# It4innovations/hyperqueue

Hardware: AMD Instinct MI355X
Metric: tasks_assigned_per_sec (higher is better)
Workload: dtype u64

## Files before the change

### hyperqueue_amd/csrc/debug_capi.cpp

```cpp
#include "../../include/hqtick_debug.h"

#include <algorithm>
#include <cstring>

#include "audit_core.h"
#include "cancel_core.h"
#include "clock_core.h"
#include "fail_core.h"
#include "finish_core.h"
#include "lose_core.h"
#include "start_core.h"
#include "reject_core.h"
#include "hb_order.h"
#include "milp.h"
#include "price_emul.h"

static thread_local int g_last_canonical = 0;
static thread_local long g_last_hull[2] = {0, 0};
extern "C" int hqtick_debug_milp_was_canonical(void) { return g_last_canonical; }
extern "C" void hqtick_debug_milp_last_hull(long *solves, long *nonpacking) {
    if (solves) *solves = g_last_hull[0];
    if (nonpacking) *nonpacking = g_last_hull[1];
}

// ... 37 lines not shown
    m.rhs.assign(rhs, rhs + nrows);
    m.roff.assign(row_off, row_off + nrows + 1);
    int nnz = nrows ? row_off[nrows] : 0;
    m.rcol.assign(row_col, row_col + nnz);
    m.rcoef.assign(row_coef, row_coef + nnz);
    if (col_group) m.col_group.assign(col_group, col_group + ncols);
    if (row_implied) m.row_implied.assign(row_implied, row_implied + nrows);
    hqprice::EmulatedSweeper emu;
    if (min_cols) emu.min_cols = min_cols;
    hqmilp::Result r = hqmilp::solve(m, time_limit_s, true, hqmilp::REFERENCE_MIP_REL_GAP, use_sweeps ? &emu : nullptr);
    g_last_canonical = r.canonical ? 1 : 0;
    g_last_hull[0] = r.hull_solves; g_last_hull[1] = r.hull_solves_nonpacking;
    if (stats_out) { stats_out[0] = r.price_sweeps; stats_out[1] = r.price_rounds; stats_out[2] = r.price_total_us; stats_out[3] = r.canonical ? 1.0 : 0.0; }
    if (!r.feasible) return 0;
    for (int j = 0; j < ncols; j++) x_out[j] = r.x[j];
    *obj_out = r.objective;
    *is_optimal = r.optimal ? 1 : 0;
    return 1;
}

static thread_local hqmilp::Probe g_block_run_probe;
extern "C" void hqtick_debug_set_block_runs(int on) {
    hqmilp::g_probe = on < 0 ? nullptr : &g_block_run_probe; hqmilp::set_block_runs(on);
    if (on >= 0) { g_block_run_probe.model = g_block_run_probe.tables = g_block_run_probe.runs = g_block_run_probe.covered = 0; }
}
extern "C" void hqtick_debug_corrupt_block_runs(int on) { g_block_run_probe.corrupt_runs = on != 0; }
extern "C" void hqtick_debug_last_coupled_digest(uint64_t out[4]) {
    out[0] = g_block_run_probe.model; out[1] = g_block_run_probe.tables; out[2] = g_block_run_probe.runs; out[3] = g_block_run_probe.covered;
}
extern "C" void hqtick_debug_set_early_sweep(int on) { hqprice::set_early_sweep(on); }
extern "C" uint32_t hqtick_debug_early_sweeps(void) { return hqprice::early_sweeps(); }
extern "C" void hqtick_debug_capture_first_cut(int on) { hqprice::capture_first_cut(on != 0); }
extern "C" uint32_t hqtick_debug_first_cut(unsigned char *out, uint32_t cap) {
    const std::vector<unsigned char> &b = hqprice::first_cut_bytes();
    if (out && cap) memcpy(out, b.data(), std::min<size_t>(cap, b.size()));
    return (uint32_t)b.size();
}

static thread_local hqmilp::CheckHook g_row_check_hook;
static hqmilp::CheckHook &row_check_hook() { hqmilp::g_check_hook = &g_row_check_hook; return g_row_check_hook; }
extern "C" void hqtick_debug_set_defer_row_check(int on) { row_check_hook().allow = on; }
extern "C" uint32_t hqtick_debug_deferred_row_checks(int clear) { hqmilp::CheckHook &h = row_check_hook(); const uint32_t n = h.deferred; if (clear) h.deferred = 0; return n; }
extern "C" uint32_t hqtick_debug_fail_row_checks(uint32_t n) { hqmilp::CheckHook &h = row_check_hook(); const uint32_t left = h.fail_next; h.fail_next = n; return left; }

extern "C" int hqtick_debug_clock_rows(uint32_t n, const int64_t *deadline_ns, int64_t now_ns, uint32_t nv, const uint64_t *min_time_ns, int sorted_form, int64_t *remaining_out) {
    if ((n && (!deadline_ns || !remaining_out)) || (nv && !min_time_ns)) return HQTICK_E_INVALID;
    if (!sorted_form) {
        for (uint32_t w = 0; w < n; w++) {
            if (deadline_ns[w] == hqclock::NO_LIMIT) { remaining_out[w] = hqclock::NO_LIMIT; continue; }
            const int64_t r = hqclock::sat_sub(deadline_ns[w], now_ns);
            uint64_t best = 0;
            for (uint32_t v0 = 0; r >= 0 && v0 < nv; v0 += hqclock::CHUNK) best = hqclock::fold_thresholds(best, r, min_time_ns + v0, std::min(hqclock::CHUNK, nv - v0));
// ... 97 lines not shown
```

### hyperqueue_amd/csrc/host_model.cpp

```cpp
#include "host_model.h"

#include <algorithm>
#include <chrono>
#include <cmath>
#include <cstring>
#include <string>
#include <unordered_map>

#include "hb_order.h"

namespace hqhost {

namespace {

struct OrderEntry { uint64_t hash = 0; bool used = false; std::vector<uint32_t> ids, order; };
thread_local OrderEntry order_cache[32];
thread_local unsigned order_next = 0;
const std::vector<uint32_t> &cached_worker_order(const std::vector<uint32_t> &ids) {
    typedef OrderEntry Entry;
    Entry (&cache)[32] = order_cache;
    unsigned &next = order_next;
    uint64_t h = 0x9E3779B97F4A7C15ull ^ ids.size();
    for (uint32_t v : ids) { h ^= v; h *= 0xFF51AFD7ED558CCDull; h ^= h >> 29; }
    for (Entry &e : cache) if (e.used && e.hash == h && e.ids.size() == ids.size() && (ids.empty() || memcmp(e.ids.data(), ids.data(), ids.size() * 4) == 0)) return e.order;
// ... 1204 lines not shown
                    list_row(hqmilp::ROW_MAX, (double)cut.size, no_gap_id, *no_gap, -1, 0.0);
                }
            }
        }
    }

    if (!seq_start.empty()) {
        m.start.assign(m.ncols(), 0.0);
        for (const SeqStart &ss : seq_start) {
            const int pc = place_get(ss.w, batches[ss.batch].rq, ss.variant);
            if (pc < 0) { m.start.clear(); break; }
            m.start[pc] = ss.count;
        }
    }
    m.row_implied.resize(m.nrows(), 0);
    m.row_lhs.resize((size_t)m.nrows(), -1); m.row_lhs_len.resize((size_t)m.nrows(), 0); m.row_block.resize((size_t)m.nrows(), -1);
    m.col_ub = col_ub; m.col_ub.resize((size_t)m.ncols(), UINT32_MAX);
    if (hqmilp::g_probe) {
        using hqmilp::fnv1a_vec;
        uint64_t h = hqmilp::FNV_BASIS;
        h = fnv1a_vec(h, m.obj); h = fnv1a_vec(h, m.kind); h = fnv1a_vec(h, m.rtype); h = fnv1a_vec(h, m.rhs); h = fnv1a_vec(h, m.roff); h = fnv1a_vec(h, m.rcol); h = fnv1a_vec(h, m.rcoef);
        h = fnv1a_vec(h, m.start); h = fnv1a_vec(h, m.col_group); h = fnv1a_vec(h, m.row_implied); h = fnv1a_vec(h, m.row_lhs); h = fnv1a_vec(h, m.row_lhs_len);
        h = fnv1a_vec(h, m.list_off); h = fnv1a_vec(h, m.list_col); h = fnv1a_vec(h, m.row_block); h = fnv1a_vec(h, m.col_ub);
        hqmilp::g_probe->model = h; hqmilp::g_probe->runs = m.block_runs.size(); hqmilp::g_probe->tables = 0; hqmilp::g_probe->covered = 0;
    }
    const double t_model1 = clock_us();
    if (trace_model) {
        size_t run_blocks = 0; for (const auto &br : m.block_runs) run_blocks += (size_t)br.n_blocks;
        fprintf(stderr, "[model] cuts done at %.3f ms: %d columns, %d rows, %zu terms, %zu worker signatures, %zu (batch, cut, blocker) passes over the workers; %zu equal-block runs over %zu blocks, %zu (cut, blocker) passes decided once\n", (t_model1 - t_model0) / 1e3, m.ncols(), m.nrows(), m.rcol.size(), sig_rep.size(), n_triples, m.block_runs.size(), run_blocks, n_decided_once);
    }
    hqmilp::SolveOpts opts; opts.no_fast_path = pb.no_fast_path; opts.defer_row_check = pb.defer_row_check;
    hqmilp::Result sol = hqmilp::solve(m, pb.time_limit_s, !pb.certificate_only, hqmilp::REFERENCE_MIP_REL_GAP, pb.pricer, &opts);
    if (trace_model) fprintf(stderr, "[model] solve done %.3f ms after the model\n", (clock_us() - t_model1) / 1e3);
    out.pre_us = t_model0 - t_enter; out.model_us = t_model1 - t_model0; out.milp_us = clock_us() - t_model1; out.price_sweeps = sol.price_sweeps; out.price_rounds = sol.price_rounds; out.price_us = sol.price_total_us;
    out.milp_nodes = sol.nodes; out.milp_cols = m.ncols(); out.milp_rows = m.nrows(); out.milp_components = sol.n_components;
    if (!sol.feasible) return out;
    out.is_optimal = sol.optimal;
    out.is_canonical = sol.canonical && sol.optimal;

    std::vector<uint64_t> key_hash; std::vector<std::pair<uint32_t, uint8_t>> key_list; std::vector<std::vector<std::pair<uint32_t, uint32_t>>> key_counts;
    std::vector<uint64_t> mn_hash; std::vector<uint32_t> mn_list; std::vector<std::vector<std::vector<uint32_t>>> mn_sets;
    std::vector<uint32_t> dec_ids, dec_widx, dec_cnt;
    for (const TaskBatch &batch : batches) {
        const RequestView &rv = pb.rqs[batch.rq];
        if (pb.rq_multi_node(batch.rq)) {
            size_t n_nodes = pb.variants[rv.first_variant].n_nodes;
            std::vector<std::vector<uint32_t>> sets;
// ... 42 lines not shown
```

### hyperqueue_amd/csrc/milp.cpp

```cpp
#include "milp.h"
#include "lp_tab.h"
#include "price.h"

#include <algorithm>
#include <chrono>
#include <cstdio>
#include <cstdlib>
#include <cmath>
#include <climits>
#include <cstring>
#include <functional>
#include <numeric>
#include <string>
#include <unordered_map>

namespace hqmilp {
namespace {

using namespace lp;

struct DSUlite {
    std::vector<int> p;
    explicit DSUlite(int n) : p(n) { std::iota(p.begin(), p.end(), 0); }
    int find(int a) { while (p[a] != a) { p[a] = p[p[a]]; a = p[a]; } return a; }
// ... 1336 lines not shown
    rc.pending = false;
    if (g_check_hook && g_check_hook->fail_next > 0) { g_check_hook->fail_next--; return false; }
    return check_point(m, rc.x, rc.cost_scale, rc.bound, rc.rel_gap, &rc.objective);
}

namespace {
bool solve_fast(const Model &mdl_in, double time_limit_s, double rel_gap, hqprice::Sweeper *sweeper, const double ts0, const SolveOpts *opts, Result &res_out) {
    static const bool tracing_solve = getenv("HQMILP_TRACE") != nullptr;
    auto tmark = [&](const char *what) { if (tracing_solve && mdl_in.ncols() > 1000) fprintf(stderr, "[milp] solve(): %s at %.3f ms\n", what, (wall() - ts0) * 1e3); };
    static const bool fast_env = !(getenv("HQMILP_FAST") && atoi(getenv("HQMILP_FAST")) == 0);
    const bool fast_on = !(opts && opts->no_fast_path) && (g_fast_path < 0 ? fast_env : g_fast_path != 0);
    const int FAST_MIN_COLS = 2048;
    const bool hints_there = (int)mdl_in.col_group.size() == mdl_in.ncols() && (int)mdl_in.row_lhs.size() == mdl_in.nrows() && (int)mdl_in.row_lhs_len.size() == mdl_in.nrows();
    const bool takes_it = fast_on && sweeper && rel_gap > 0.0 && mdl_in.ncols() >= FAST_MIN_COLS && mdl_in.ncols() >= (int)sweeper->min_cols && hints_there && (int)mdl_in.start.size() != mdl_in.ncols();
    if (takes_it || (g_probe && hints_there)) {
        const int n = mdl_in.ncols(), m = mdl_in.nrows();
        hqprice::ModelView mv;
        mv.n = n; mv.m = m; mv.obj = mdl_in.obj.data(); mv.kind = mdl_in.kind.data(); mv.rtype = mdl_in.rtype.data(); mv.rhs = mdl_in.rhs.data();
        mv.roff = mdl_in.roff.data(); mv.rcol = mdl_in.rcol.data(); mv.rcoef = mdl_in.rcoef.data(); mv.col_group = mdl_in.col_group.data();
        mv.row_implied = (int)mdl_in.row_implied.size() == m ? mdl_in.row_implied.data() : nullptr; mv.row_lhs = mdl_in.row_lhs.data(); mv.row_lhs_len = mdl_in.row_lhs_len.data(); mv.list_off = mdl_in.list_off.data(); mv.list_col = mdl_in.list_col.data(); mv.n_lists = (int)mdl_in.list_off.size() - 1;
        if ((int)mdl_in.row_block.size() == m && (int)mdl_in.col_ub.size() == n) { mv.row_block = mdl_in.row_block.data(); mv.col_ub = mdl_in.col_ub.data(); }
        static_assert(sizeof(Model::BlockRun) == 7 * sizeof(int32_t), "ModelView::block_runs reads seven int32 per run");
        if (!mdl_in.block_runs.empty()) { mv.block_runs = &mdl_in.block_runs[0].col0; mv.n_block_runs = (int)mdl_in.block_runs.size(); }
        mv.run_stats = g_probe ? &g_probe->covered : nullptr; mv.tables_digest = g_probe ? &g_probe->tables : nullptr;
        if (!takes_it) { hqprice::flatten_for_probe(mv, tracing_solve); return false; }
        double cost_scale = 1.0;
        const double tf0 = wall();
        hqprice::Answer pa = hqprice::solve_model(mv, rel_gap, time_limit_s, ts0 + (time_limit_s > 0 ? time_limit_s : 1e18), tracing_solve, *sweeper, &cost_scale);
        if (tracing_solve) fprintf(stderr, "[milp] fast path: ran %d (%s) sweeps %u rounds %u bound %.9f point %.9f, %.3f ms of which %.3f ms inside the sweeps\n", (int)pa.ran, pa.why, pa.sweeps, pa.rounds, pa.ran ? pa.bound : -1.0, pa.x.empty() ? -1.0 : pa.x_value, (wall() - tf0) * 1e3, sweeper->stat_sweep_us / 1e3);
        if (pa.ran && (int)pa.x.size() == n && pa.bound * (1.0 + 1e-9) + 1e-12 <= pa.x_value + rel_gap * std::fabs(pa.x_value)) {
            if (opts && opts->defer_row_check) {
                Result res;
                res.x.resize((size_t)n);
                for (int j = 0; j < n; j++) res.x[(size_t)j] = std::floor(pa.x[(size_t)j] + 0.5);
                res.feasible = true; res.optimal = true; res.canonical = false;
                res.n_components = 1; res.nodes = pa.sweeps; res.price_sweeps = (int)pa.sweeps; res.price_rounds = (int)pa.rounds; res.price_total_us = (wall() - tf0) * 1e6;
                res.row_check.pending = true; res.row_check.x = std::move(pa.x); res.row_check.cost_scale = cost_scale; res.row_check.bound = pa.bound; res.row_check.rel_gap = rel_gap;
                if (g_check_hook) g_check_hook->deferred++;
                tmark("fast path certified by the sweeps, row check pending");
                res_out = std::move(res);
                return true;
            }
            double z_pt = 0.0;
            const bool ok = check_point(mdl_in, pa.x, cost_scale, pa.bound, rel_gap, &z_pt);
            if (ok) {
                Result res;
                res.x = std::move(pa.x);
// ... 301 lines not shown
```

### hyperqueue_amd/csrc/milp.h

```cpp
#pragma once
#include <cstddef>
#include <cstdint>
#include <algorithm>
#include <vector>

namespace hqprice { struct Sweeper; }

namespace hqmilp {

enum { COL_NAT = 0, COL_BOOL = 1 };
enum { ROW_MIN = 0, ROW_MAX = 1, ROW_EQ = 2 };

struct Model {
    std::vector<double> obj;
    std::vector<uint8_t> kind;
    std::vector<uint8_t> rtype;
    std::vector<double> rhs;
    std::vector<int> roff{0};
    std::vector<int> rcol;
    std::vector<double> rcoef;
    std::vector<double> start;
    std::vector<int32_t> col_group;
    std::vector<uint8_t> row_implied;
    std::vector<int32_t> row_lhs, row_lhs_len;
// ... 60 lines not shown
    int n_components = 0;
    int price_sweeps = 0, price_rounds = 0;
    double price_bound_us = 0, price_total_us = 0;
    long hull_solves = 0, hull_solves_nonpacking = 0;
    RowCheck row_check;
};

struct SolveOpts {
    bool no_fast_path = false;
    bool defer_row_check = false;
};

const double REFERENCE_MIP_REL_GAP = 1e-4;

Result solve(const Model &m, double time_limit_s, bool canonical = true, double rel_gap = REFERENCE_MIP_REL_GAP, hqprice::Sweeper *sweeper = nullptr, const SolveOpts *opts = nullptr);

bool check_point(const Model &m, const std::vector<double> &x, double cost_scale, double bound, double rel_gap, double *objective);
bool run_row_check(const Model &m, RowCheck &rc);

void columns_by_cost_desc(const double *c, int n, std::vector<int> &out);
void set_fast_path(int on);
void set_block_runs(int on);
bool block_runs_on();
struct Probe { uint64_t model = 0, tables = 0, runs = 0, covered = 0; bool corrupt_runs = false; };
extern thread_local Probe *g_probe;
struct CheckHook { int allow = -1; uint32_t deferred = 0, fail_next = 0; };
extern thread_local CheckHook *g_check_hook;
inline uint64_t fnv1a(uint64_t h, const void *p, size_t bytes) { const unsigned char *b = (const unsigned char *)p; for (size_t i = 0; i < bytes; i++) h = (h ^ b[i]) * 1099511628211ull; return h; }
template <class T> inline uint64_t fnv1a_vec(uint64_t h, const std::vector<T> &v) { const uint64_t n = v.size(); h = fnv1a(h, &n, 8); return v.empty() ? h : fnv1a(h, v.data(), v.size() * sizeof(T)); }
const uint64_t FNV_BASIS = 1469598103934665603ull;

}
```

### hyperqueue_amd/csrc/price.cpp

```cpp
#include "price_prob.h"

#include <algorithm>
#include <chrono>
#include <cmath>
#include <cstdio>
#include <cstdlib>
#include <cstring>
#include <functional>
#include <map>
#include <numeric>

#include "lp_tab.h"
#include "milp.h"

namespace hqprice {
namespace {

using hqmilp::lp::BASIC;
using hqmilp::lp::INF;
using hqmilp::lp::LP_OPT;
using hqmilp::lp::Rows;
using hqmilp::lp::Tab;

static_assert(UNBOUNDED == INF, "price_prob.h restates lp_tab.h's INF");
// ... 649 lines not shown
        out.lambda.assign(cuts.size(), 0.0); out.bfrac.assign(G, 0.0);
        double lsum = 0.0;
        for (int r = 0; r < M.m; r++) {
            const int a = mt.where[r];
            if (a < 0 || mt.st[M.n + a] == BASIC) continue;
            const double v = std::fabs(mt.d[M.n + a]) / row_scale[r];
            if (row_cut[r] >= 0) { out.lambda[row_cut[r]] = v; lsum += v; } else out.bfrac[freeg[r]] = std::min(1.0, v);
        }
        for (int g = 0; g < G; g++) if (nd.flag[g] >= 0) out.bfrac[g] = (double)nd.flag[g];
        if (lsum > 0.0) for (double &l : out.lambda) l /= lsum; else out.lambda.clear();
        out.pi.assign(mt.x.begin(), mt.x.begin() + K);
    }
};

}

namespace {
thread_local bool g_capture_cut = false; thread_local std::vector<unsigned char> g_first_cut;
Answer run_solver(Solver &S, const double tp0) {
    Answer ans;
    const Request &rq = S.rq; Sweeper &sw = S.sw;
    auto tmark = [&](const char *what) { if (rq.trace) fprintf(stderr, "[price] %s at %.3f ms (sweeps so far %.3f ms)\n", what, (now_us() - tp0) / 1e3, sw.stat_sweep_us / 1e3); };
    tmark("model flattened");
    if (rq.trace) fprintf(stderr, "[price]   %d equal-block runs took %d of %u blocks from their first one\n", S.P.n_runs, S.P.run_blocks, S.P.T.n_blocks);
    Prob &P = S.P;
    if (rq.trace) fprintf(stderr, "[price] %u blocks, %u block columns, %d wide rows with %d distinct left-hand sides (%zu / %zu terms), %d flags, %zu conditional bounds\n", P.T.n_blocks, P.T.n_cols, P.K, P.KG, P.row_terms, P.T.w_row.size(), P.G, P.caps.size());
    const int K = P.K, G = P.G;
    struct Ender { Sweeper *s; ~Ender() { if (s) s->end(); } } ender{S.early_begun ? &sw : nullptr};
    std::vector<double> pi0(K, 0.0);
    if (S.early == Solver::EARLY_REFUSED) { ans.why = "sweeper refused the model"; return ans; }
    if (S.early == Solver::EARLY_FAILED) { S.failed = true; ans.why = "sweep failed"; return ans; }
    if (S.early == Solver::EARLY_LAUNCHED) {
        if (!sw.begin_wide()) { ans.why = "sweeper refused the model"; return ans; }
        tmark("wide tables handed to the sweeper");
    } else {
        S.prepare_sweeper();
        if (!sw.begin(P.T, (uint32_t)S.max_sweeps)) { ans.why = "sweeper refused the model"; return ans; }
        ender.s = &sw;
        tmark("tables handed to the sweeper");
        if (!S.evaluate_launch(pi0)) { ans.why = "sweep failed"; return ans; }
    }
    S.pmax.assign(K, 0.0);
    {
        double cmax = 0.0; for (double c : P.T.col_cost) cmax = std::max(cmax, c);
        std::vector<double> gp(P.KG, 0.0);
        for (int g = 0; g < P.KG; g++) {
            double p = 0.0; bool neg = false; int32_t amin = INT32_MAX;
// ... 344 lines not shown
```

### hyperqueue_amd/csrc/price.h

```cpp
#pragma once
#include <cstdint>
#include <functional>
#include <vector>

namespace hqprice {

struct HostTables {
    uint32_t n_blocks = 0, n_cols = 0, K = 0;
    std::vector<uint32_t> blk_off; std::vector<uint8_t> blk_m; std::vector<double> blk_cap;
    std::vector<double> col_cost, col_a; std::vector<int32_t> col_cap; std::vector<uint32_t> col_woff; std::vector<uint16_t> w_row; std::vector<int32_t> w_coef;
};

struct SweepTotals {
    double cx = 0, rc = 0, bnd = 0;
    uint32_t n_budget = 0, max_steps = 0;
    std::vector<long long> act;
    std::vector<double> part_cx;
    std::vector<long long> part_act;
};
constexpr int PARTS = 16;

struct RangeValues { const double *cx = nullptr, *rc = nullptr, *bnd = nullptr; const uint32_t *steps = nullptr; const long long *part_act = nullptr; };

void totals_from_blocks(uint32_t n_blocks, uint32_t K, const double *cx, const double *rc, const double *bnd, const uint32_t *steps, const long long *part_act, SweepTotals &out);
// ... 39 lines not shown
    bool ran = false;
    double bound = 1e300;
    std::vector<double> x;
    double x_value = 0.0;
    uint32_t sweeps = 0, rounds = 0;
    const char *why = "";
    std::vector<int> block_of; std::vector<double> block_value, rcost;
};

Answer solve(const Request &rq, Sweeper &sw);

struct ModelView {
    int n = 0, m = 0;
    const double *obj = nullptr; const uint8_t *kind = nullptr;
    const uint8_t *rtype = nullptr; const double *rhs = nullptr;
    const int *roff = nullptr, *rcol = nullptr; const double *rcoef = nullptr;
    const int32_t *col_group = nullptr; const uint8_t *row_implied = nullptr;
    const int32_t *row_lhs = nullptr, *row_lhs_len = nullptr;
    const int *list_off = nullptr, *list_col = nullptr; int n_lists = 0;
    const int32_t *row_block = nullptr; const uint32_t *col_ub = nullptr;
    const int32_t *block_runs = nullptr; int n_block_runs = 0;
    uint64_t *run_stats = nullptr;
    uint64_t *tables_digest = nullptr;
};
void set_check_hints(bool on);
int hint_mismatches();
void set_early_sweep(int on);
uint32_t early_sweeps();
void capture_first_cut(bool on);
const std::vector<unsigned char> &first_cut_bytes();
void flatten_for_probe(const ModelView &mv, bool trace);
Answer solve_model(const ModelView &mv, double rel_gap, double time_limit_s, double deadline_s, bool trace, Sweeper &sw, double *cost_scale);

struct Exchange {
    uint32_t rank = 0, world = 1;
    virtual ~Exchange() {}
    virtual bool allgather(const void *send, void *recv, size_t bytes) = 0;
    uint64_t n_calls = 0, n_bytes = 0; double us = 0;
};

struct ShardedSweeper : Sweeper {
    Sweeper &inner; Exchange &ex;
    const HostTables *T = nullptr;
    std::vector<uint32_t> rank_b0, rank_b1, rank_p0, rank_p1;
    uint32_t max_blocks = 0, max_parts = 0, max_cols = 0;
    std::vector<unsigned char> send, recv;
    std::vector<double> cx, rc, bnd; std::vector<uint32_t> steps; std::vector<long long> part_act;
// ... 16 lines not shown
```

### hyperqueue_amd/csrc/price_flatten.cpp

```cpp
#include "price_prob.h"

#include <cstdio>
#include <cstring>

#include "milp.h"

namespace hqprice {
namespace {

constexpr double INF = UNBOUNDED;
thread_local bool g_check_hints = false; thread_local int g_hint_mismatches = 0;

#define HQ_PER_ROW inline __attribute__((always_inline))

typedef std::vector<std::pair<int, int32_t>> Lhs;

void finish_groups(Prob &P, const std::vector<Lhs> &lhs) {
    HostTables &T = P.T;
    const int KG = P.KG;
    T.K = (uint32_t)KG;
    size_t tot = 0; for (auto &l : lhs) tot += l.size();
    P.g_off.assign((size_t)KG + 1, 0); P.g_col.resize(tot); P.g_coef.resize(tot);
    std::vector<uint32_t> gcnt(T.n_cols + 1, 0);
    {
        auto *gc = P.g_col.data(); auto *gk = P.g_coef.data(); uint32_t *cnt = gcnt.data() + 1; size_t pos = 0;
        for (int g = 0; g < KG; g++) {
            const std::pair<int, int32_t> *l = lhs[(size_t)g].data();
            for (size_t i = 0, e = lhs[(size_t)g].size(); i < e; i++) { gc[pos] = l[i].first; gk[pos] = l[i].second; cnt[l[i].first]++; pos++; }
            P.g_off[(size_t)g + 1] = (int)pos;
        }
    }
    T.col_woff.assign(T.n_cols + 1, 0);
    for (uint32_t f = 0; f < T.n_cols; f++) T.col_woff[f + 1] = T.col_woff[f] + gcnt[f + 1];
    T.w_row.resize(T.col_woff[T.n_cols]); T.w_coef.resize(T.col_woff[T.n_cols]);
    {
        std::vector<uint32_t> &cur = gcnt;
        for (uint32_t f = 0; f < T.n_cols; f++) cur[f] = T.col_woff[f];
        uint32_t *cp = cur.data(); uint16_t *wr = T.w_row.data(); auto *wc = T.w_coef.data();
        const auto *gc = P.g_col.data(); const auto *gk = P.g_coef.data();
        for (int g = 0; g < KG; g++) for (int e = P.g_off[g], e1 = P.g_off[g + 1]; e < e1; e++) { const uint32_t p = cp[gc[e]]++; wr[p] = (uint16_t)g; wc[p] = gk[e]; }
    }
    P.gr_off.assign((size_t)KG + 1, 0);
    for (int k = 0; k < P.K; k++) P.gr_off[P.grp_of[k] + 1]++;
    for (int g = 0; g < KG; g++) P.gr_off[g + 1] += P.gr_off[g];
    P.gr_row.resize(P.K);
    { std::vector<int> c2(P.gr_off.begin(), P.gr_off.end() - 1); for (int k = 0; k < P.K; k++) P.gr_row[c2[P.grp_of[k]]++] = k; }
}

struct Scan { int b0 = -2; bool multi = false, has_g = false, nonneg = true; int n_bcols = 0; double amax = 0.0; };
struct Row { int a = 0, e = 0; bool is_le = false, is_ge = false, implied = false; double lo = 0.0, hi = 0.0; int list = -1, list_len = 0; Scan sc; };
struct WideRow { double h; uint8_t ge; int lhs_key; int own = -1; std::vector<std::pair<int, double>> g; };

template <class Rnd> HQ_PER_ROW const char *grid_terms(const double *coef, int nt, double scale, Rnd rnd, long long *vi, long long &g) {
    g = 0;
    for (int k = 0; k < nt; k++) {
        const double v = coef[k] * scale * GRID, rv = rnd(v);
        if (rv < 1.0 || std::fabs(v - rv) > 1e-6 * std::max(1.0, rv) || rv >= 4.0e15) return "block row off the ResourceAmount grid";
        vi[k] = (long long)rv;
        g = gcd_ll(g, vi[k]);
    }
    return nullptr;
}

struct Core {
    Prob &P; HostTables &T;
    const int n; const int32_t *const col_group; const int *const rcol; const double *const rcoef;
    const double *ub = nullptr, *c = nullptr;
    int max_group = -1, nb = 0;
    std::vector<int> block_of_group, bsize, blk, gidx;
    std::vector<WideRow> wide;
    std::vector<Lhs> own_lists;

    Core(Prob &p, int n_, const int32_t *cg, const int *rc, const double *rv) : P(p), T(p.T), n(n_), col_group(cg), rcol(rc), rcoef(rv) {}

    const char *number_blocks() {
        for (int j = 0; j < n; j++) max_group = std::max(max_group, col_group[j]);
        block_of_group.assign((size_t)max_group + 1, -1); blk.assign(n, -1);
        for (int j = 0; j < n; j++) {
            const int g = col_group[j];
            if (g < 0) { P.gmodel.push_back(j); continue; }
            if (block_of_group[g] < 0) { block_of_group[g] = (int)bsize.size(); bsize.push_back(0); }
            blk[j] = block_of_group[g];
            if (++bsize[blk[j]] > NMAX_BLOCK) return "block with more than 32 columns";
        }
        nb = (int)bsize.size();
        if (nb < 8) return "fewer than 8 blocks";
        return nullptr;
    }
    template <class Is01> const char *take_globals(Is01 is01) {
        P.G = (int)P.gmodel.size();
        for (int j : P.gmodel) {
            if (!is01(j)) return "global column that is not 0/1";
            if (c[j] < 0.0) return "global column with negative cost";
            P.gcost.push_back(c[j]);
// ... 83 lines not shown
            if (!own) return "block column behind a shared list";
            const double rv = Src::rnd(v);
            if (std::fabs(v - rv) > 1e-7 * std::max(1.0, std::fabs(rv)) || std::fabs(rv) > 1.0e9) return "wide row with a non-integer coefficient";
            if (rv != 0.0) own->push_back({P.flat_of[j], (int32_t)rv});
        }
        P.row_terms += (size_t)(e - a) - w.g.size() + (size_t)row.list_len;
        wide.push_back(std::move(w));
        if ((int)wide.size() > 1024) return "more than 1024 wide rows";
        return nullptr;
    }

    const char *finish(const int *list_off, const int *list_col, int n_lists, const std::function<void()> *after_blocks) {
        for (int b = 0; b < nb; b++) if (T.blk_m[b] == 0) {
            double total = 0.0;
            for (uint32_t f = T.blk_off[b]; f < T.blk_off[b + 1]; f++) { T.col_a[(size_t)f * MMAX_BLOCK] = 1.0; total += (double)T.col_cap[f]; }
            T.blk_cap[(size_t)b * MMAX_BLOCK] = total;
            T.blk_m[b] = 1;
        }
        if (after_blocks && *after_blocks) (*after_blocks)();
        P.K = (int)wide.size();
        if (P.K == 0) return "no wide row";
        P.h.resize(P.K); P.ge.resize(P.K); P.g_rows.assign(P.G, {});
        P.grp_of.assign(P.K, -1);
        std::vector<Lhs> lhs;
        std::vector<uint64_t> lhs_hash;
        std::vector<int> group_of_key((size_t)2 * n_lists, -1);
        auto materialise = [&](int key, Lhs &out) {
            const int l = key >> 1;
            const int32_t sign = (key & 1) ? -1 : 1;
            const int k0 = list_off[l], k1 = list_off[l + 1];
            out.resize((size_t)(k1 - k0));
            std::pair<int, int32_t> *o = out.data(); const int *fo = P.flat_of.data();
            for (int k = k0; k < k1; k++) o[k - k0] = {fo[list_col[k]], sign};
        };
        auto hash_of = [](const Lhs &l) { uint64_t h = 1469598103934665603ull; for (auto &t : l) h = (h ^ ((uint64_t)(uint32_t)t.first | ((uint64_t)(uint32_t)t.second << 32))) * 1099511628211ull; return h; };
        Lhs tmp;
        for (int k = 0; k < P.K; k++) {
            WideRow &w = wide[(size_t)k];
            P.h[k] = w.h; P.ge[k] = w.ge;
            for (auto &t : w.g) P.g_rows[t.first].push_back({k, t.second});
            if (w.lhs_key >= 0 && group_of_key[(size_t)w.lhs_key] >= 0) { P.grp_of[k] = group_of_key[(size_t)w.lhs_key]; continue; }
            Lhs *l;
            if (w.lhs_key >= 0) { materialise(w.lhs_key, tmp); l = &tmp; } else l = &own_lists[(size_t)w.own];
            const uint64_t hsh = hash_of(*l);
            int g = -1;
            for (size_t i = 0; i < lhs.size() && g < 0; i++) if (lhs_hash[i] == hsh && lhs[i] == *l) g = (int)i;
            if (g < 0) { g = (int)lhs.size(); lhs.push_back(std::move(*l)); lhs_hash.push_back(hsh); }
            if (w.lhs_key >= 0) group_of_key[(size_t)w.lhs_key] = g;
            P.grp_of[k] = g;
        }
        P.KG = (int)lhs.size();
        if (P.KG > KMAX_HOST) return "more than 128 distinct wide left-hand sides";
        finish_groups(P, lhs);
        P.base_cap = T.col_cap;
        return nullptr;
    }
};

struct RequestRows {
    const Request &rq;
    double sc = 1.0;
    std::vector<long long> vi; std::vector<double> scaled;
    static double rnd(double v) { return std::round(v); }
    HQ_PER_ROW const char *grid(const Row &row, const double *&out, long long &g) {
        const int nt = row.e - row.a;
        vi.resize((size_t)nt); scaled.resize((size_t)nt);
        if (const char *why = grid_terms(rq.rcoef + row.a, nt, sc, [](double v) { return rnd(v); }, vi.data(), g)) return why;
        if (g < 1) g = 1;
        for (int k = 0; k < nt; k++) scaled[(size_t)k] = (double)(vi[(size_t)k] / g);
        out = scaled.data();
        return nullptr;
    }
    void fifth_row(const Row &row, int b0) const {
        if (!rq.trace) return;
        fprintf(stderr, "[price] 5th row of block %d: hi %.6f scale %.6f:", b0, row.hi, sc);
        for (int k = row.a; k < row.e; k++) fprintf(stderr, " %.6f*x%d(ub %.0f)", rq.rcoef[k] * sc, rq.rcol[k], rq.ub[rq.rcol[k]]);
// ... 176 lines not shown
                    if (blk[j] < 0) { f.sc.has_g = true; continue; }
                    f.sc.n_bcols++;
                    if (f.sc.b0 == -2) f.sc.b0 = blk[j]; else if (blk[j] != f.sc.b0) f.sc.multi = true;
                }
            }
            if (!(f.sc.multi && !f.sc.has_g)) return "shared list that is not a wide left-hand side";
            sc = f.sc;
            row.list = L; row.list_len = f.len;
        }
        const int hint_b = (hinted && L < 0 && mv.row_block[i] >= 0 && mv.row_block[i] <= max_group) ? block_of_group[mv.row_block[i]] : -1;
        if (hint_b >= 0) {
            if (row.implied) continue;
            sc.b0 = hint_b; sc.n_bcols = e - a;
            const int32_t hb = mv.row_block[i];
            for (int k = a; k < e; k++) {
                if (mv.col_group[mv.rcol[k]] != hb) return "structure hint: a row_block row holds a column of another block";
                if (mv.rcoef[k] < 0.0) sc.nonneg = false;
                sc.amax += mv.rcoef[k] * ub[mv.rcol[k]];
            }
        } else F.scan(a, e, sc);
        if (const char *why = F.place(src, row)) return why;
    }
    if (run_live) stamp_run(runs[run_i]);
    return F.finish(mv.list_off, mv.list_col, n_lhs, after_blocks);
}

}

const char *flatten(const Request &rq, Prob &P) {
    if (!rq.col_group) return "no block hints";
    Core F(P, rq.n, rq.col_group, rq.rcol, rq.rcoef);
    F.ub = rq.ub; F.c = rq.c;
    if (const char *why = F.number_blocks()) return why;
    if (const char *why = F.take_globals([&](int j) { return rq.ub[j] == 1.0; })) return why;
    if (const char *why = F.alloc_tables()) return why;
    RequestRows src{rq};
    for (int i = 0; i < rq.m; i++) {
        Row row; row.a = rq.roff[i]; row.e = rq.roff[i + 1];
        if (row.a == row.e) continue;
        src.sc = rq.row_scale[i];
        row.is_le = rq.rlo[i] <= -INF; row.is_ge = rq.rhi[i] >= INF;
        row.lo = rq.rlo[i]; row.hi = rq.rhi[i];
        row.implied = rq.row_implied && rq.row_implied[i];
        F.scan(row.a, row.e, row.sc);
        if (const char *why = F.place(src, row)) return why;
    }
// ... 5 lines not shown
    const HostTables &T = P.T;
    uint64_t h = hqmilp::FNV_BASIS;
    const uint32_t dims[3] = {T.n_blocks, T.n_cols, T.K}; h = fnv1a(h, dims, sizeof dims);
    h = fnv1a_vec(h, T.blk_off); h = fnv1a_vec(h, T.blk_m); h = fnv1a_vec(h, T.blk_cap); h = fnv1a_vec(h, T.col_cost); h = fnv1a_vec(h, T.col_a); h = fnv1a_vec(h, T.col_cap);
    h = fnv1a_vec(h, T.col_woff); h = fnv1a_vec(h, T.w_row); h = fnv1a_vec(h, T.w_coef);
    const int dims2[3] = {P.K, P.G, P.KG}; h = fnv1a(h, dims2, sizeof dims2);
    h = fnv1a_vec(h, P.h); h = fnv1a_vec(h, P.ge); h = fnv1a_vec(h, P.grp_of); h = fnv1a_vec(h, P.g_off); h = fnv1a_vec(h, P.g_col); h = fnv1a_vec(h, P.g_coef);
    h = fnv1a_vec(h, P.gr_off); h = fnv1a_vec(h, P.gr_row); h = fnv1a_vec(h, P.gmodel); h = fnv1a_vec(h, P.gcost); h = fnv1a_vec(h, P.flat_of); h = fnv1a_vec(h, P.model_of);
    h = fnv1a_vec(h, P.block_of_flat); h = fnv1a_vec(h, P.base_cap);
    for (const CapRow &cr : P.caps) { h = fnv1a(h, &cr.flat, sizeof cr.flat); h = fnv1a(h, &cr.rhs, sizeof cr.rhs); for (auto &t : cr.g) { h = fnv1a(h, &t.first, sizeof t.first); h = fnv1a(h, &t.second, sizeof t.second); } }
    for (const auto &gr : P.g_rows) { const uint64_t nn = gr.size(); h = fnv1a(h, &nn, 8); for (auto &t : gr) { h = fnv1a(h, &t.first, sizeof t.first); h = fnv1a(h, &t.second, sizeof t.second); } }
    return h;
}

const char *flatten(const ModelView &mv, Prob &P, std::vector<double> &ub, std::vector<double> &c, double &cmax, const std::function<void()> *after_blocks) {
    const char *why = flatten_once(mv, P, ub, c, cmax, after_blocks);
    if (!why && g_check_hints && mv.block_runs) {
        ModelView plain = mv; plain.block_runs = nullptr; plain.n_block_runs = 0;
        Prob P2; std::vector<double> ub2, c2; double cmax2 = 0.0;
        const char *why2 = flatten_once(plain, P2, ub2, c2, cmax2, nullptr);
        if (why2 || digest_of(P2) != digest_of(P) || ub2 != ub || c2 != c || cmax2 != cmax) { g_hint_mismatches++; return "structure hint: a block run's tables differ from its blocks' own"; }
    }
    if (!why && mv.run_stats) *mv.run_stats += (uint64_t)P.run_blocks;
    if (!why && mv.tables_digest) *mv.tables_digest = digest_of(P);
    return why;
}

void flatten_for_probe(const ModelView &mv, bool trace) {
    Prob P; std::vector<double> ub, c; double cmax = 1.0;
    const char *why = flatten(mv, P, ub, c, cmax);
    if (trace) fprintf(stderr, "[price] flattened for the probe alone: %s\n", why ? why : "tables built");
}

void set_check_hints(bool on) { g_check_hints = on; g_hint_mismatches = 0; }
int hint_mismatches() { return g_hint_mismatches; }

}
```

### hyperqueue_amd/csrc/price_prob.h

```cpp
#pragma once
#include "price.h"

#include <algorithm>
#include <cmath>
#include <utility>

namespace hqprice {

constexpr int KMAX_HOST = 128;
constexpr int NMAX_BLOCK = 32, MMAX_BLOCK = 4;
constexpr double GRID = 10000.0;
constexpr double UNBOUNDED = 1e300;

struct CapRow { int flat; double rhs; std::vector<std::pair<int, double>> g; };

struct Prob {
    HostTables T;
    std::vector<int> flat_of, model_of;
    std::vector<int> gmodel;
    std::vector<double> gcost;
    int K = 0, G = 0;
    std::vector<double> h;
    std::vector<uint8_t> ge;
    std::vector<std::vector<std::pair<int, double>>> g_rows;
    std::vector<int> grp_of;
    int KG = 0;
    std::vector<int> g_off, g_col; std::vector<int32_t> g_coef;
    std::vector<int> gr_off, gr_row;
    size_t row_terms = 0;
    std::vector<CapRow> caps;
    std::vector<int32_t> base_cap;
    std::vector<int> block_of_flat;
    int n_runs = 0, run_blocks = 0;
};

inline double round_fast(double v) { return (double)(long long)(v + (v >= 0.0 ? 0.5 : -0.5)); }
inline long long gcd_ll(long long a, long long b) { while (b) { const long long t = a % b; a = b; b = t; } return a < 0 ? -a : a; }

const char *flatten(const Request &rq, Prob &P);
const char *flatten(const ModelView &mv, Prob &P, std::vector<double> &ub, std::vector<double> &c, double &cmax, const std::function<void()> *after_blocks = nullptr);
uint64_t digest_of(const Prob &P);

struct Polisher {
    const Prob &P; int n;
    explicit Polisher(const Prob &p, int n_) : P(p), n(n_) {}
    bool run(std::vector<double> &x, double &value) const {
        const HostTables &T = P.T; const int K = P.K, G = P.G;
        if ((int)x.size() != n) return false;
        std::vector<double> xf(T.n_cols), B(G);
        for (uint32_t f = 0; f < T.n_cols; f++) { const double v = x[P.model_of[f]], rv = round_fast(v); if (v < -1e-9 || v > (double)P.base_cap[f] + 1e-9 || std::fabs(v - rv) > 1e-9) return false; xf[f] = rv; }
        for (int g = 0; g < G; g++) { B[g] = x[P.gmodel[g]]; if (B[g] != 0.0 && B[g] != 1.0) return false; }
        std::vector<double> bact((size_t)T.n_blocks * MMAX_BLOCK, 0.0);
        for (uint32_t b = 0; b < T.n_blocks; b++) {
            double *ba = &bact[(size_t)b * MMAX_BLOCK];
            for (uint32_t f = T.blk_off[b]; f < T.blk_off[b + 1]; f++) if (xf[f] != 0.0) for (int r = 0; r < MMAX_BLOCK; r++) ba[r] += T.col_a[(size_t)f * MMAX_BLOCK + r] * xf[f];
            for (int r = 0; r < (int)T.blk_m[b]; r++) if (ba[r] > T.blk_cap[(size_t)b * MMAX_BLOCK + r]) return false;
// ... 51 lines not shown
```

### include/hqtick_debug.h

```cpp
#ifndef HQTICK_DEBUG_H
#define HQTICK_DEBUG_H
#include <stdint.h>
#include "hqtick.h"
#ifdef __cplusplus
extern "C" {
#endif
#if defined(__GNUC__)
#pragma GCC visibility push(default)
#endif

int hqtick_debug_milp_solve(int ncols, const double *obj, const uint8_t *col_kind, int nrows, const uint8_t *row_type,
                            const double *rhs, const int *row_off, const int *row_col, const double *row_coef,
                            double time_limit_s, int canonical, double *x_out, double *obj_out, int *is_optimal,
                            long *nodes_out);

int hqtick_debug_last_order(const hqtick_ctx *ctx, uint32_t *n_runs, uint32_t *n_levels, double *order_us);

int hqtick_debug_last_scan(const hqtick_ctx *ctx, int which, uint32_t *n_levels, uint32_t *n_groups, uint32_t shape[4],
                           uint64_t *levels, uint32_t cap_levels, uint32_t *hist, uint32_t cap_groups);

int hqtick_debug_order_view(hqtick_ctx *ctx, uint32_t n_requests, uint32_t counts[4], uint32_t *perm, uint32_t *inv, uint32_t *lrank, uint64_t cap_slots, uint32_t *run_rq,
                            uint32_t *run_start, uint32_t *run_rank, uint64_t *run_prio, uint32_t cap_runs);
int hqtick_debug_order_select(hqtick_ctx *ctx, const uint32_t *rq_sel_base, const uint32_t *q_tnc, uint32_t n_sel, int mark_mode, uint64_t *sel_task, uint32_t *sel_rank,
                              uint32_t *rq_after, uint32_t *err);
// ... 14 lines not shown
void hqtick_debug_milp_last_hull(long *solves, long *nonpacking);

void hqtick_debug_map_order_u32(const uint32_t *keys, uint32_t n, uint32_t *out_pos);

int hqtick_debug_block_solve_host(uint32_t n_cols, uint32_t n_resources, const uint32_t *ent_off, const uint32_t *ent_res, const uint8_t *ent_kind,
                                  const uint64_t *ent_amount, const uint32_t *weight, const double *pool, uint32_t n_classes, const uint64_t *free_,
                                  const uint64_t *total, const uint64_t *elig, uint32_t budget, uint32_t *x, uint32_t *status, uint32_t *steps);
void hqtick_debug_set_block_emulation(int on, uint32_t budget);
void hqtick_debug_last_stage_us(double *out3);
void hqtick_debug_last_blocks(uint32_t *n_emulated, uint32_t *n_host);

int hqtick_time_kernel(hqtick_ctx *ctx, int which, int iters, double *avg_us);
int hqtick_timeline(const hqtick_ctx *ctx, double *out, int cap);
const uint64_t *hqtick_block_profile_last(const hqtick_ctx *ctx, uint32_t *n_classes);


void hqtick_debug_set_price_emulation(int on, uint32_t min_cols);
void hqtick_debug_set_price_fault(int fail_at);
void hqtick_debug_set_fast_path(int on);
void hqtick_debug_check_model_hints(int on);
int hqtick_debug_model_hint_mismatches(void);
void hqtick_debug_set_block_runs(int on);
void hqtick_debug_last_coupled_digest(uint64_t out[4]);
void hqtick_debug_set_early_sweep(int on);
uint32_t hqtick_debug_early_sweeps(void);
void hqtick_debug_set_defer_row_check(int on);
uint32_t hqtick_debug_deferred_row_checks(int clear);
uint32_t hqtick_debug_fail_row_checks(uint32_t n);
void hqtick_debug_capture_first_cut(int on);
uint32_t hqtick_debug_first_cut(unsigned char *out, uint32_t cap);
void hqtick_debug_corrupt_block_runs(int on);
void hqtick_debug_last_price(uint32_t *sweeps, uint32_t *rounds);
uint32_t hqtick_debug_last_mn(const uint32_t **rq, const uint32_t **off, const uint32_t **worker);
int hqtick_debug_milp_solve_priced(int ncols, const double *obj, const uint8_t *col_kind, const int32_t *col_group, int nrows, const uint8_t *row_type,
                                   const uint8_t *row_implied, const double *rhs, const int *row_off, const int *row_col, const double *row_coef,
                                   double time_limit_s, int use_sweeps, uint32_t min_cols, double *x_out, double *obj_out, int *is_optimal, double *stats_out);

struct hqwire_tables;
struct hqwire_records;
struct hqwire_output;
int hqwire_debug_encode_host(const struct hqwire_tables *tables, const struct hqwire_records *records, const struct hqwire_output *out);
int hqwire_debug_encode_host_order(const struct hqwire_tables *tables, const struct hqwire_records *records, const struct hqwire_output *out, int order);
struct hqwire_table;
struct hqwire_table_config;
int hqwire_debug_table_create_host(struct hqwire_table **out, const struct hqwire_table_config *cfg, int order);

// ... 56 lines not shown
```

Measured before the change: 70.65 million.

## Reuse equal-block runs when flattening wide-row left-hand sides in pricer

When building the pricer's wide-row tables, left-hand sides are now cut into pieces that align with runs of identical blocks. Only the first block of each run is counted and scattered, and the offsets and entries for the remaining blocks are replicated by arithmetic and memcpy. Pure run-structured left-hand sides are deduplicated by a compact descriptor instead of materialising and hashing the full term list. This is meant to cut host-side flattening cost on models with many repeated blocks, at the price of more complex grouping code and fallback paths when a run turns out irregular. It is on by default and can be disabled through an environment variable or a debug toggle.

Measured after the change: 74.13 million (median of 6 runs). 1.05x the previous value.

```diff
diff --git a/hyperqueue_amd/csrc/debug_capi.cpp b/hyperqueue_amd/csrc/debug_capi.cpp
--- a/hyperqueue_amd/csrc/debug_capi.cpp
+++ b/hyperqueue_amd/csrc/debug_capi.cpp
@@ -83,12 +83,14 @@
 static thread_local hqmilp::Probe g_block_run_probe;
 extern "C" void hqtick_debug_set_block_runs(int on) {
     hqmilp::g_probe = on < 0 ? nullptr : &g_block_run_probe; hqmilp::set_block_runs(on);
-    if (on >= 0) { g_block_run_probe.model = g_block_run_probe.tables = g_block_run_probe.runs = g_block_run_probe.covered = 0; }
+    if (on >= 0) { g_block_run_probe.model = g_block_run_probe.tables = g_block_run_probe.runs = g_block_run_probe.covered = g_block_run_probe.wide = 0; }
 }
 extern "C" void hqtick_debug_corrupt_block_runs(int on) { g_block_run_probe.corrupt_runs = on != 0; }
 extern "C" void hqtick_debug_last_coupled_digest(uint64_t out[4]) {
     out[0] = g_block_run_probe.model; out[1] = g_block_run_probe.tables; out[2] = g_block_run_probe.runs; out[3] = g_block_run_probe.covered;
 }
+extern "C" void hqtick_debug_set_wide_runs(int on) { hqprice::set_wide_runs(on); }
+extern "C" uint64_t hqtick_debug_last_wide_blocks(void) { return g_block_run_probe.wide; }
 extern "C" void hqtick_debug_set_early_sweep(int on) { hqprice::set_early_sweep(on); }
 extern "C" uint32_t hqtick_debug_early_sweeps(void) { return hqprice::early_sweeps(); }
 extern "C" void hqtick_debug_capture_first_cut(int on) { hqprice::capture_first_cut(on != 0); }
diff --git a/hyperqueue_amd/csrc/host_model.cpp b/hyperqueue_amd/csrc/host_model.cpp
--- a/hyperqueue_amd/csrc/host_model.cpp
+++ b/hyperqueue_amd/csrc/host_model.cpp
@@ -1250,7 +1250,7 @@
         h = fnv1a_vec(h, m.obj); h = fnv1a_vec(h, m.kind); h = fnv1a_vec(h, m.rtype); h = fnv1a_vec(h, m.rhs); h = fnv1a_vec(h, m.roff); h = fnv1a_vec(h, m.rcol); h = fnv1a_vec(h, m.rcoef);
         h = fnv1a_vec(h, m.start); h = fnv1a_vec(h, m.col_group); h = fnv1a_vec(h, m.row_implied); h = fnv1a_vec(h, m.row_lhs); h = fnv1a_vec(h, m.row_lhs_len);
         h = fnv1a_vec(h, m.list_off); h = fnv1a_vec(h, m.list_col); h = fnv1a_vec(h, m.row_block); h = fnv1a_vec(h, m.col_ub);
-        hqmilp::g_probe->model = h; hqmilp::g_probe->runs = m.block_runs.size(); hqmilp::g_probe->tables = 0; hqmilp::g_probe->covered = 0;
+        hqmilp::g_probe->model = h; hqmilp::g_probe->runs = m.block_runs.size(); hqmilp::g_probe->tables = 0; hqmilp::g_probe->covered = 0; hqmilp::g_probe->wide = 0;
     }
     const double t_model1 = clock_us();
     if (trace_model) {
diff --git a/hyperqueue_amd/csrc/milp.cpp b/hyperqueue_amd/csrc/milp.cpp
--- a/hyperqueue_amd/csrc/milp.cpp
+++ b/hyperqueue_amd/csrc/milp.cpp
@@ -1382,7 +1382,7 @@
         if ((int)mdl_in.row_block.size() == m && (int)mdl_in.col_ub.size() == n) { mv.row_block = mdl_in.row_block.data(); mv.col_ub = mdl_in.col_ub.data(); }
         static_assert(sizeof(Model::BlockRun) == 7 * sizeof(int32_t), "ModelView::block_runs reads seven int32 per run");
         if (!mdl_in.block_runs.empty()) { mv.block_runs = &mdl_in.block_runs[0].col0; mv.n_block_runs = (int)mdl_in.block_runs.size(); }
-        mv.run_stats = g_probe ? &g_probe->covered : nullptr; mv.tables_digest = g_probe ? &g_probe->tables : nullptr;
+        mv.run_stats = g_probe ? &g_probe->covered : nullptr; mv.tables_digest = g_probe ? &g_probe->tables : nullptr; mv.wide_stats = g_probe ? &g_probe->wide : nullptr;
         if (!takes_it) { hqprice::flatten_for_probe(mv, tracing_solve); return false; }
         double cost_scale = 1.0;
         const double tf0 = wall();
diff --git a/hyperqueue_amd/csrc/milp.h b/hyperqueue_amd/csrc/milp.h
--- a/hyperqueue_amd/csrc/milp.h
+++ b/hyperqueue_amd/csrc/milp.h
@@ -106,7 +106,7 @@
 void set_fast_path(int on);
 void set_block_runs(int on);
 bool block_runs_on();
-struct Probe { uint64_t model = 0, tables = 0, runs = 0, covered = 0; bool corrupt_runs = false; };
+struct Probe { uint64_t model = 0, tables = 0, runs = 0, covered = 0; bool corrupt_runs = false; uint64_t wide = 0; };
 extern thread_local Probe *g_probe;
 struct CheckHook { int allow = -1; uint32_t deferred = 0, fail_next = 0; };
 extern thread_local CheckHook *g_check_hook;
diff --git a/hyperqueue_amd/csrc/price.cpp b/hyperqueue_amd/csrc/price.cpp
--- a/hyperqueue_amd/csrc/price.cpp
+++ b/hyperqueue_amd/csrc/price.cpp
@@ -695,7 +695,7 @@
     const Request &rq = S.rq; Sweeper &sw = S.sw;
     auto tmark = [&](const char *what) { if (rq.trace) fprintf(stderr, "[price] %s at %.3f ms (sweeps so far %.3f ms)\n", what, (now_us() - tp0) / 1e3, sw.stat_sweep_us / 1e3); };
     tmark("model flattened");
-    if (rq.trace) fprintf(stderr, "[price]   %d equal-block runs took %d of %u blocks from their first one\n", S.P.n_runs, S.P.run_blocks, S.P.T.n_blocks);
+    if (rq.trace) fprintf(stderr, "[price]   %d equal-block runs took %d of %u blocks from their first one; %d runs gave %d blocks their wide-row entries\n", S.P.n_runs, S.P.run_blocks, S.P.T.n_blocks, S.P.wide_runs, S.P.wide_blocks);
     Prob &P = S.P;
     if (rq.trace) fprintf(stderr, "[price] %u blocks, %u block columns, %d wide rows with %d distinct left-hand sides (%zu / %zu terms), %d flags, %zu conditional bounds\n", P.T.n_blocks, P.T.n_cols, P.K, P.KG, P.row_terms, P.T.w_row.size(), P.G, P.caps.size());
     const int K = P.K, G = P.G;
diff --git a/hyperqueue_amd/csrc/price.h b/hyperqueue_amd/csrc/price.h
--- a/hyperqueue_amd/csrc/price.h
+++ b/hyperqueue_amd/csrc/price.h
@@ -85,7 +85,9 @@
     const int32_t *block_runs = nullptr; int n_block_runs = 0;
     uint64_t *run_stats = nullptr;
     uint64_t *tables_digest = nullptr;
+    uint64_t *wide_stats = nullptr;
 };
+void set_wide_runs(int on);
 void set_check_hints(bool on);
 int hint_mismatches();
 void set_early_sweep(int on);
diff --git a/hyperqueue_amd/csrc/price_flatten.cpp b/hyperqueue_amd/csrc/price_flatten.cpp
--- a/hyperqueue_amd/csrc/price_flatten.cpp
+++ b/hyperqueue_amd/csrc/price_flatten.cpp
@@ -1,6 +1,7 @@
 #include "price_prob.h"
 
 #include <cstdio>
+#include <cstdlib>
 #include <cstring>
 
 #include "milp.h"
@@ -10,35 +11,138 @@
 
 constexpr double INF = UNBOUNDED;
 thread_local bool g_check_hints = false; thread_local int g_hint_mismatches = 0;
+thread_local int g_wide_runs = -1;
+bool wide_runs_on() {
+    static const bool env_on = !(getenv("HQPRICE_WIDE_RUNS") && atoi(getenv("HQPRICE_WIDE_RUNS")) == 0);
+    return g_wide_runs < 0 ? env_on : g_wide_runs != 0;
+}
 
 #define HQ_PER_ROW inline __attribute__((always_inline))
 
 typedef std::vector<std::pair<int, int32_t>> Lhs;
 
-void finish_groups(Prob &P, const std::vector<Lhs> &lhs) {
+struct WideRun { int col0, f0, nbk, nc; };
+struct Piece { int start, len, run, t; };
+struct Cut { std::vector<Piece> pieces; bool pure = false; std::vector<int32_t> desc; int n_terms = 0; };
+struct Group { Lhs lhs; int key = -1; Cut cut; uint64_t hash = 0; };
+
+struct WideRuns {
+    std::vector<WideRun> runs;
+    std::vector<uint8_t> bad;
+    std::vector<uint8_t> seen;
+    int last = 0;
+    bool on() const { return !runs.empty(); }
+    template <bool MODEL> int run_of(int j) {
+        auto lo = [](const WideRun &r) { return MODEL ? r.col0 : r.f0; };
+        { const WideRun &r = runs[(size_t)last]; if (j >= lo(r) && j < lo(r) + r.nbk * r.nc) return last; }
+        int a = 0, b = (int)runs.size();
+        while (b - a > 1) { const int mid = (a + b) / 2; if (lo(runs[(size_t)mid]) <= j) a = mid; else b = mid; }
+        const WideRun &r = runs[(size_t)a];
+        if (j < lo(r) || j >= lo(r) + r.nbk * r.nc) return -1;
+        return last = a;
+    }
+    template <bool MODEL, class Col, class Coef> void cut_lhs(int n, Col col, Coef coef, Cut &out) {
+        out.pieces.clear(); out.desc.clear(); out.pure = true; out.n_terms = n;
+        std::fill(seen.begin(), seen.end(), 0);
+        int plain0 = -1;
+        auto plain = [&](int k) { out.pure = false; if (plain0 < 0) plain0 = k; };
+        auto flush = [&](int k) { if (plain0 >= 0) { out.pieces.push_back({plain0, k - plain0, -1, 0}); plain0 = -1; } };
+        int k = 0;
+        while (k < n) {
+            const int j = col(k), r = run_of<MODEL>(j);
+            if (r < 0) { plain(k); k++; continue; }
+            const WideRun &R = runs[(size_t)r];
+            const int base = MODEL ? R.col0 : R.f0;
+            if (seen[(size_t)r] || j - base >= R.nc) { bad[(size_t)r] = 1; seen[(size_t)r] = 1; plain(k); k++; continue; }
+            seen[(size_t)r] = 1;
+            int t = 1;
+            while (k + t < n && col(k + t) >= base && col(k + t) < base + R.nc) t++;
+            const long long need = (long long)R.nbk * t;
+            bool ok = (long long)k + need <= n;
+            if (ok) for (int i = k, e = k + (int)need - t; i < e; i++) ok &= col(i + t) == col(i) + R.nc && coef(i + t) == coef(i);
+            if (!ok) { bad[(size_t)r] = 1; plain(k); k += t; continue; }
+            flush(k);
+            out.pieces.push_back({k, (int)need, r, t});
+            out.desc.push_back(r); out.desc.push_back(t);
+            for (int i = 0; i < t; i++) { out.desc.push_back(col(k + i) - base); out.desc.push_back(coef(k + i)); }
+            k += (int)need;
+        }
+        flush(n);
+    }
+};
+
+void finish_groups(Prob &P, const std::vector<Group> &groups, const WideRuns &wr_, const int *list_off, const int *list_col) {
     HostTables &T = P.T;
     const int KG = P.KG;
     T.K = (uint32_t)KG;
-    size_t tot = 0; for (auto &l : lhs) tot += l.size();
+    size_t tot = 0; for (auto &g : groups) tot += (size_t)g.cut.n_terms;
     P.g_off.assign((size_t)KG + 1, 0); P.g_col.resize(tot); P.g_coef.resize(tot);
+    {
+        auto *gc = P.g_col.data(); auto *gk = P.g_coef.data(); size_t pos = 0;
+        for (int g = 0; g < KG; g++) {
+            const Group &G = groups[(size_t)g];
+            if (G.key < 0) {
+                const std::pair<int, int32_t> *l = G.lhs.data();
+                for (size_t i = 0, e = G.lhs.size(); i < e; i++) { gc[pos + i] = l[i].first; gk[pos + i] = l[i].second; }
+            } else {
+                const int32_t sign = (G.key & 1) ? -1 : 1;
+                const int *lc = list_col + list_off[G.key >> 1]; const int *fo = P.flat_of.data();
+                for (const Piece &p : G.cut.pieces) {
+                    const int nc = wr_.runs[(size_t)p.run].nc, nbk = wr_.runs[(size_t)p.run].nbk;
+                    int *o = gc + pos + p.start;
+                    for (int i = 0; i < p.t; i++) o[i] = fo[lc[p.start + i]];
+                    for (int b = 1; b < nbk; b++) for (int i = 0; i < p.t; i++) o[b * p.t + i] = o[i] + b * nc;
+                }
+                for (int i = 0; i < G.cut.n_terms; i++) gk[pos + i] = sign;
+            }
+            pos += (size_t)G.cut.n_terms;
+            P.g_off[(size_t)g + 1] = (int)pos;
+        }
+    }
+    auto taken = [&](const Piece &p) { return p.run >= 0 && !wr_.bad[(size_t)p.run] ? p.t : p.len; };
     std::vector<uint32_t> gcnt(T.n_cols + 1, 0);
     {
-        auto *gc = P.g_col.data(); auto *gk = P.g_coef.data(); uint32_t *cnt = gcnt.data() + 1; size_t pos = 0;
-        for (int g = 0; g < KG; g++) {
-            const std::pair<int, int32_t> *l = lhs[(size_t)g].data();
-            for (size_t i = 0, e = lhs[(size_t)g].size(); i < e; i++) { gc[pos] = l[i].first; gk[pos] = l[i].second; cnt[l[i].first]++; pos++; }
-            P.g_off[(size_t)g + 1] = (int)pos;
-        }
+        const auto *gc = P.g_col.data(); uint32_t *cnt = gcnt.data() + 1;
+        for (int g = 0; g < KG; g++) for (const Piece &p : groups[(size_t)g].cut.pieces) { const int *c = gc + P.g_off[g] + p.start; for (int i = 0, e = taken(p); i < e; i++) cnt[c[i]]++; }
     }
     T.col_woff.assign(T.n_cols + 1, 0);
-    for (uint32_t f = 0; f < T.n_cols; f++) T.col_woff[f + 1] = T.col_woff[f] + gcnt[f + 1];
+    {
+        uint32_t *wo = T.col_woff.data(); const uint32_t *cnt = gcnt.data() + 1;
+        size_t ri = 0; const size_t nr = wr_.runs.size();
+        uint32_t f = 0;
+        while (f < T.n_cols) {
+            while (ri < nr && (wr_.bad[ri] || (uint32_t)wr_.runs[ri].f0 < f)) ri++;
+            const uint32_t stop = ri < nr ? (uint32_t)wr_.runs[ri].f0 : T.n_cols;
+            for (; f < stop; f++) wo[f + 1] = wo[f] + cnt[f];
+            if (f == T.n_cols) break;
+            const WideRun &R = wr_.runs[ri];
+            const uint32_t nc = (uint32_t)R.nc;
+            for (uint32_t q = 0; q < nc; q++) wo[f + q + 1] = wo[f + q] + cnt[f + q];
+            const uint32_t W = wo[f + nc] - wo[f];
+            for (uint32_t k = 1; k < (uint32_t)R.nbk; k++) for (uint32_t q = 1; q <= nc; q++) wo[f + k * nc + q] = wo[f + q] + k * W;
+            f += (uint32_t)R.nbk * nc; ri++;
+        }
+    }
     T.w_row.resize(T.col_woff[T.n_cols]); T.w_coef.resize(T.col_woff[T.n_cols]);
     {
         std::vector<uint32_t> &cur = gcnt;
         for (uint32_t f = 0; f < T.n_cols; f++) cur[f] = T.col_woff[f];
         uint32_t *cp = cur.data(); uint16_t *wr = T.w_row.data(); auto *wc = T.w_coef.data();
         const auto *gc = P.g_col.data(); const auto *gk = P.g_coef.data();
-        for (int g = 0; g < KG; g++) for (int e = P.g_off[g], e1 = P.g_off[g + 1]; e < e1; e++) { const uint32_t p = cp[gc[e]]++; wr[p] = (uint16_t)g; wc[p] = gk[e]; }
+        for (int g = 0; g < KG; g++) for (const Piece &pc : groups[(size_t)g].cut.pieces) {
+            const int e0 = P.g_off[g] + pc.start;
+            for (int e = e0, e1 = e0 + taken(pc); e < e1; e++) { const uint32_t p = cp[gc[e]]++; wr[p] = (uint16_t)g; wc[p] = gk[e]; }
+        }
+        for (size_t ri = 0; ri < wr_.runs.size(); ri++) if (!wr_.bad[ri]) {
+            const WideRun &R = wr_.runs[ri];
+            const size_t s = T.col_woff[(size_t)R.f0], W = T.col_woff[(size_t)R.f0 + (size_t)R.nc] - s, total = W * (size_t)R.nbk;
+            for (size_t filled = W; filled < total && W > 0; ) {
+                const size_t n = std::min(filled, total - filled);
+                memcpy(wr + s + filled, wr + s, n * sizeof(uint16_t)); memcpy(wc + s + filled, wc + s, n * sizeof(int32_t));
+                filled += n;
+            }
+            P.wide_runs++; P.wide_blocks += R.nbk - 1;
+        }
     }
     P.gr_off.assign((size_t)KG + 1, 0);
     for (int k = 0; k < P.K; k++) P.gr_off[P.grp_of[k] + 1]++;
@@ -70,6 +174,7 @@
     std::vector<int> block_of_group, bsize, blk, gidx;
     std::vector<WideRow> wide;
     std::vector<Lhs> own_lists;
+    WideRuns W;
 
     Core(Prob &p, int n_, const int32_t *cg, const int *rc, const double *rv) : P(p), T(p.T), n(n_), col_group(cg), rcol(rc), rcoef(rv) {}
 
@@ -199,9 +304,10 @@
         if (P.K == 0) return "no wide row";
         P.h.resize(P.K); P.ge.resize(P.K); P.g_rows.assign(P.G, {});
         P.grp_of.assign(P.K, -1);
-        std::vector<Lhs> lhs;
-        std::vector<uint64_t> lhs_hash;
+        std::vector<Group> groups;
         std::vector<int> group_of_key((size_t)2 * n_lists, -1);
+        Cut cut;
+        W.bad.assign(W.runs.size(), 0); W.seen.assign(W.runs.size(), 0); W.last = 0;
         auto materialise = [&](int key, Lhs &out) {
             const int l = key >> 1;
             const int32_t sign = (key & 1) ? -1 : 1;
@@ -217,18 +323,34 @@
             P.h[k] = w.h; P.ge[k] = w.ge;
             for (auto &t : w.g) P.g_rows[t.first].push_back({k, t.second});
             if (w.lhs_key >= 0 && group_of_key[(size_t)w.lhs_key] >= 0) { P.grp_of[k] = group_of_key[(size_t)w.lhs_key]; continue; }
-            Lhs *l;
-            if (w.lhs_key >= 0) { materialise(w.lhs_key, tmp); l = &tmp; } else l = &own_lists[(size_t)w.own];
-            const uint64_t hsh = hash_of(*l);
+            Lhs *l = w.lhs_key >= 0 ? nullptr : &own_lists[(size_t)w.own];
+            if (!W.on()) {
+                cut.n_terms = l ? (int)l->size() : list_off[(w.lhs_key >> 1) + 1] - list_off[w.lhs_key >> 1];
+                cut.pieces.assign(1, Piece{0, cut.n_terms, -1, 0});
+            } else if (l) {
+                const std::pair<int, int32_t> *t = l->data();
+                W.cut_lhs<false>((int)l->size(), [t](int i) { return t[i].first; }, [t](int i) { return t[i].second; }, cut);
+            } else {
+                const int *lc = list_col + list_off[w.lhs_key >> 1];
+                const int32_t sign = (w.lhs_key & 1) ? -1 : 1;
+                W.cut_lhs<true>(list_off[(w.lhs_key >> 1) + 1] - list_off[w.lhs_key >> 1], [lc](int i) { return lc[i]; }, [sign](int) { return sign; }, cut);
+            }
             int g = -1;
-            for (size_t i = 0; i < lhs.size() && g < 0; i++) if (lhs_hash[i] == hsh && lhs[i] == *l) g = (int)i;
-            if (g < 0) { g = (int)lhs.size(); lhs.push_back(std::move(*l)); lhs_hash.push_back(hsh); }
+            if (cut.pure) {
+                for (size_t i = 0; i < groups.size() && g < 0; i++) if (groups[i].cut.pure && groups[i].cut.desc == cut.desc) g = (int)i;
+                if (g < 0) { g = (int)groups.size(); groups.emplace_back(); Group &G = groups.back(); G.cut = cut; if (l) G.lhs = std::move(*l); else G.key = w.lhs_key; }
+            } else {
+                if (!l) { materialise(w.lhs_key, tmp); l = &tmp; }
+                const uint64_t hsh = hash_of(*l);
+                for (size_t i = 0; i < groups.size() && g < 0; i++) if (!groups[i].cut.pure && groups[i].hash == hsh && groups[i].lhs == *l) g = (int)i;
+                if (g < 0) { g = (int)groups.size(); groups.emplace_back(); Group &G = groups.back(); G.cut = cut; G.hash = hsh; G.lhs = std::move(*l); }
+            }
             if (w.lhs_key >= 0) group_of_key[(size_t)w.lhs_key] = g;
             P.grp_of[k] = g;
         }
-        P.KG = (int)lhs.size();
+        P.KG = (int)groups.size();
         if (P.KG > KMAX_HOST) return "more than 128 distinct wide left-hand sides";
-        finish_groups(P, lhs);
+        finish_groups(P, groups, W, list_off, list_col);
         P.base_cap = T.col_cap;
         return nullptr;
     }
@@ -451,6 +573,7 @@
         if (const char *why = F.place(src, row)) return why;
     }
     if (run_live) stamp_run(runs[run_i]);
+    if (wide_runs_on()) for (const Run &R : runs) F.W.runs.push_back({R.col0, (int)T.blk_off[R.b0], R.nbk, R.nc});
     return F.finish(mv.list_off, mv.list_col, n_lhs, after_blocks);
 }
 
@@ -502,6 +625,7 @@
         if (why2 || digest_of(P2) != digest_of(P) || ub2 != ub || c2 != c || cmax2 != cmax) { g_hint_mismatches++; return "structure hint: a block run's tables differ from its blocks' own"; }
     }
     if (!why && mv.run_stats) *mv.run_stats += (uint64_t)P.run_blocks;
+    if (!why && mv.wide_stats) *mv.wide_stats += (uint64_t)P.wide_blocks;
     if (!why && mv.tables_digest) *mv.tables_digest = digest_of(P);
     return why;
 }
@@ -512,6 +636,7 @@
     if (trace) fprintf(stderr, "[price] flattened for the probe alone: %s\n", why ? why : "tables built");
 }
 
+void set_wide_runs(int on) { g_wide_runs = on; }
 void set_check_hints(bool on) { g_check_hints = on; g_hint_mismatches = 0; }
 int hint_mismatches() { return g_hint_mismatches; }
 
diff --git a/hyperqueue_amd/csrc/price_prob.h b/hyperqueue_amd/csrc/price_prob.h
--- a/hyperqueue_amd/csrc/price_prob.h
+++ b/hyperqueue_amd/csrc/price_prob.h
@@ -32,6 +32,7 @@
     std::vector<int32_t> base_cap;
     std::vector<int> block_of_flat;
     int n_runs = 0, run_blocks = 0;
+    int wide_runs = 0, wide_blocks = 0;
 };
 
 inline double round_fast(double v) { return (double)(long long)(v + (v >= 0.0 ? 0.5 : -0.5)); }
diff --git a/include/hqtick_debug.h b/include/hqtick_debug.h
--- a/include/hqtick_debug.h
+++ b/include/hqtick_debug.h
@@ -60,6 +60,8 @@
 int hqtick_debug_model_hint_mismatches(void);
 void hqtick_debug_set_block_runs(int on);
 void hqtick_debug_last_coupled_digest(uint64_t out[4]);
+void hqtick_debug_set_wide_runs(int on);
+uint64_t hqtick_debug_last_wide_blocks(void);
 void hqtick_debug_set_early_sweep(int on);
 uint32_t hqtick_debug_early_sweeps(void);
 void hqtick_debug_set_defer_row_check(int on);
```
